# kmacrow/Shellac

Measured on AMD Instinct MI355X. Metric: cache_ops_per_s, higher is better.
Workload: dtype uint8

## Files before the change

shellac_amd/csrc/hbm_cache.h:

```cpp
#pragma once

#include <hip/hip_runtime_api.h>

#include <algorithm>
#include <mutex>
#include <string>
#include <vector>

#include "layout.h"

namespace shellac {

enum : int { kEvictFifo = 0, kEvictClock = 1 };

struct ShardConfig {
  uint64_t log_bytes = 1ull << 30;
  uint64_t nbuckets = 1ull << 20;
  uint32_t max_item = 1u << 20;
  int device = 0;
  int evict = kEvictClock;
  uint64_t reinsert_max = 0;
  int serve_blocks = 8;
};

// ... 117 lines not shown
  void ensure_set_ws(int64_t n, hipStream_t s);
  void ensure_rc_ws(int64_t w, hipStream_t s);
  void ensure_cb(int b, int64_t rows, hipStream_t s);
  bool should_reclaim(uint64_t bytes_bound) const;
  uint64_t* cur_ring_tail() const { return head_ + 2 + hsel_; }
  uint64_t* next_ring_tail() const { return head_ + 2 + (hsel_ ^ 1); }
  struct RetiredGroup {
    std::vector<void*> ptrs;
    std::vector<hipEvent_t> ev;
    uint64_t bytes = 0;
  };
  struct Buf {
    void** p;
    uint64_t (*bytes)(uint64_t cap);
  };
  using BufSet = std::vector<Buf>;
  void grow_bufs(const BufSet& set, int64_t old_cap, int64_t cap, hipStream_t s);
  void retire_group(const BufSet& set, int64_t cap, hipStream_t s);
  void reap_retired(bool all);
  void note_stream(hipStream_t s);
  void note_store_end(hipStream_t s);
  std::vector<RetiredGroup> retired_;
  uint64_t retired_ever_ = 0;
  struct SetStream {
    hipStream_t s = nullptr;
    hipEvent_t last = nullptr;
  };
  std::vector<SetStream> set_streams_;
  hipEvent_t ws_ready_ = nullptr;
  hipStream_t ws_grow_stream_ = nullptr;
  std::vector<hipStream_t> ws_ordered_;
  void ws_order(hipStream_t s);
  uint64_t* ring_ = nullptr;
  uint64_t ring_cap_ = 0;
  unsigned long long* rc_ctl_ = nullptr;
  bool lead_ = false;
  bool catch_up_ = true;
  uint64_t rmax_ = 0;
  int64_t rc_cap_ = 0;
  uint64_t *rc_loc_ = nullptr, *rc_h_ = nullptr, *rc_part_ = nullptr, *rc_hx_ = nullptr;
  BufSet rc_bufs();
  struct Pending {
    const Digest* keys = nullptr;
    const uint8_t* values = nullptr;
    const uint64_t* voff = nullptr;
    const uint32_t *vlen = nullptr, *flags = nullptr, *expire = nullptr;
    int64_t n = 0, rows = 0;
    const uint64_t* from = nullptr;
    int64_t nmove = 0;
    int ws = 0;
    int hand = -1;
    bool active = false;
  };
  Pending pend_;
  struct HandBuf {
    Digest* keys = nullptr;
    uint64_t* voff = nullptr;
    uint64_t* from = nullptr;
    uint32_t *vlen = nullptr, *flags = nullptr, *expire = nullptr;
    int64_t cap = 0;
    uint8_t* scratch = nullptr;
  };
  HandBuf hb_[2];
  static BufSet hand_bufs(HandBuf& h);
  struct SetWs {
    uint32_t* dd_tab = nullptr;
    uint32_t* dd_slot = nullptr;
    uint64_t *set_size = nullptr, *set_off = nullptr;
    uint32_t* set_claim = nullptr;
    uint64_t* set_cnt = nullptr;
  };
  SetWs ws_[2];
  int ws_next_ = 0;
  static BufSet set_bufs(SetWs& w);

  ShardConfig cfg_;
  uint8_t* log_ = nullptr;
  Entry* index_ = nullptr;
  uint64_t* head_ = nullptr;
  int hsel_ = 0;
  uint64_t* cur_head() const { return head_ + hsel_; }
  uint64_t* claim_ptr() const { return head_ + 4; }
  uint64_t* next_head() const { return head_ + (hsel_ ^ 1); }
  CacheCounters* ctr_ = nullptr;
  unsigned long long* scratch_ = nullptr;
  uint64_t* part_ = nullptr;
  uint64_t* host_buf_ = nullptr;
  uint64_t* host_slots_ = nullptr;
  void* srv_ring_ = nullptr;
  uint64_t* srv_ctl_ = nullptr;
  uint64_t* srv_sync_ = nullptr;
// ... 74 lines not shown
```

shellac_amd/csrc/hbm_cache.hip:

```cpp
#include <hip/hip_runtime.h>
#include <hip/hip_ext.h>
#include <hipcub/hipcub.hpp>

#include <algorithm>
#include <chrono>
#include <cstdlib>
#include <cstring>
#include <type_traits>
#include <vector>

#include "hbm_cache.h"
#include "keyed.h"
#include "trace.h"

namespace shellac {

#define HIP_OK(expr)                                                                   \
  do {                                                                                 \
    hipError_t _e = (expr);                                                            \
    if (_e != hipSuccess)                                                              \
      throw Error(std::string("HIP error ") + hipGetErrorString(_e) + " at " + #expr + \
                  " [" + __FILE__ + ":" + std::to_string(__LINE__) + "]");             \
  } while (0)

// ... 1647 lines not shown
    const uint64_t e2 = __shfl(w2[2], gbase + (target & 3));
    const uint64_t expected = target < 4 ? e1 : e2;
    Entry* const slot = index + (target < 4 ? b1 : b2) * kEntriesPerBucket + (target & 3);
    int ok = 0;
    if (l4 == 0) {
      const unsigned long long prev = atomicCAS(
          reinterpret_cast<unsigned long long*>(&slot->loc), (unsigned long long)expected,
          (unsigned long long)myloc);
      if (prev == expected) {
        slot->d0 = d.lo;
        slot->d1 = d.hi;
        *reinterpret_cast<uint64_t*>(&slot->vlen) = pack2(myvlen, myexp);
        *claim_out = (uint32_t)(slot - index);
        ok = 1;
        evicted += evict ? 1 : 0;
        bytes += myvlen;
      } else if (alt != ~0ull) {
        undo_relocation(index, alt, expected);
      }
    }
    ok = __shfl(ok, gbase);
    if (ok) break;
    if (attempt == 15 && l4 == 0) ++lost;
  }
}

__global__ __launch_bounds__(kBlock) __attribute__((amdgpu_waves_per_eu(8))) void k_set_index(
    const Digest* __restrict__ keys, int64_t n, const uint64_t* __restrict__ size,
    const uint64_t* __restrict__ off, const uint32_t* __restrict__ vlen,
    const uint32_t* __restrict__ expire, Entry* __restrict__ index, uint64_t mask,
    const uint64_t* __restrict__ head_ptr, uint64_t* __restrict__ head_next, uint64_t cap,
    uint32_t now, const uint32_t* __restrict__ slot_of, uint32_t* __restrict__ dd_tab,
    CacheCounters* __restrict__ ctr, uint32_t* __restrict__ claim,
    const uint64_t* __restrict__ from, int64_t r0, int64_t r1,
    const unsigned long long* __restrict__ r1_dev) {
  if (r1_dev && (int64_t)*r1_dev < r1) r1 = (int64_t)*r1_dev;
  const int l4 = threadIdx.x & 3;
  const int gbase = threadIdx.x & 60;
  const uint64_t base = *head_ptr;
  const uint64_t head_new = base + off[n];
  const int64_t ngroups = ((int64_t)gridDim.x * kBlock) >> 2;
  unsigned long long evicted = 0, bytes = 0, lost = 0, moved_away = 0;
  if (blockIdx.x == 0 && threadIdx.x == 0) *head_next = head_new;
  for (int64_t i = r0 + (((int64_t)blockIdx.x * kBlock + threadIdx.x) >> 2); i < r1; i += ngroups) {
    if (l4 == 0 && vlen[i] != kSkipVlen) dd_tab[slot_of[i]] = 0u;
    if (l4 == 0) claim[i] = ~0u;
    if (size[i] == 0) continue;
    const Digest d = keys[i];
    const uint64_t myloc = base + off[i] + 1;
    const uint32_t myvlen = vlen[i];
    const uint32_t myexp = expire ? expire[i] : 0u;
    const uint64_t fr = from ? from[i] : 0ull;
    const uint64_t b1 = bucket1(d, mask), b2 = bucket2(d, mask);
    const uint64_t* q1 = reinterpret_cast<const uint64_t*>(index + b1 * kEntriesPerBucket + l4);
    const uint64_t* q2 = reinterpret_cast<const uint64_t*>(index + b2 * kEntriesPerBucket + l4);
    for (int attempt = 0; attempt < 16; ++attempt) {
      uint64_t w1[4], w2[4];
#pragma unroll
      for (int k = 0; k < 4; ++k) {
        w1[k] = __hip_atomic_load(q1 + k, __ATOMIC_RELAXED, __HIP_MEMORY_SCOPE_AGENT);
        w2[k] = __hip_atomic_load(q2 + k, __ATOMIC_RELAXED, __HIP_MEMORY_SCOPE_AGENT);
      }
      const uint64_t span = head_new - base;
      const bool in1 = w1[2] - base - 1 < span || w1[2] == kLockedLoc;
      const bool in2 = w2[2] - base - 1 < span || w2[2] == kLockedLoc;
      const bool m1 = w1[0] == d.lo && w1[1] == d.hi && !in1;
      const bool m2 = w2[0] == d.lo && w2[1] == d.hi && !in2;
      const bool v1 = !entry_free(w1[2], (uint32_t)(w1[3] >> 32), head_new, cap, now);
      const bool v2 = !entry_free(w2[2], (uint32_t)(w2[3] >> 32), head_new, cap, now);
      const uint32_t mmask = (uint32_t)((__ballot(m1) >> gbase) & 0xfull) |
                             ((uint32_t)((__ballot(m2) >> gbase) & 0xfull) << 4);
      const uint32_t lmask = (uint32_t)((__ballot(v1) >> gbase) & 0xfull) |
                             ((uint32_t)((__ballot(v2) >> gbase) & 0xfull) << 4);
      int target;
      if (fr) {
        const uint32_t fmask = (uint32_t)((__ballot(w1[2] == fr) >> gbase) & 0xfull) |
                               ((uint32_t)((__ballot(w2[2] == fr) >> gbase) & 0xfull) << 4);
        if (!fmask) {
          if (l4 == 0) ++moved_away;
          break;
        }
        target = __ffs(fmask) - 1;
      } else if (mmask) {
        target = __ffs(mmask) - 1;
      } else {
        const uint32_t dead = ~lmask & 0xffu;
        if (dead) {
          const int live1 = __popc(lmask & 0xfu), live2 = __popc(lmask & 0xf0u);
          const uint32_t pref = __popc(dead & 0x0fu) >= 2
                                    ? (dead & 0x0fu)
                                    : (live2 < live1 ? (dead & 0xf0u) : (dead & 0x0fu));
          target = __ffs(pref ? pref : dead) - 1;
        } else {
          if (l4 == 0) claim[i] = kClaimDeferred;
          break;
        }
      }
      const uint64_t e1 = __shfl(w1[2], gbase + (target & 3));
      const uint64_t e2 = __shfl(w2[2], gbase + (target & 3));
      const uint64_t expected = target < 4 ? e1 : e2;
      Entry* const slot = index + (target < 4 ? b1 : b2) * kEntriesPerBucket + (target & 3);
      int ok = 0;
// ... 68 lines not shown
          const uint64_t aw = agent_load(reinterpret_cast<const uint64_t*>(&a->vlen));
          if (!entry_free(al, (uint32_t)(aw >> 32), head_new, cap, now)) continue;
          if (copy_entry(a, al, de.lo, de.hi, l, w)) {
            target = x;
            expected = l;
            copy = a;
          }
          break;
        }
      }
      if (!target && victim) {
        target = victim;
        expected = oldest;
        evict = true;
      }
    }
    if (!target) continue;
    if (copy_entry(target, expected, d.lo, d.hi, myloc, myword)) {
      *claim_out = (uint32_t)(target - index);
      evicted += evict ? 1 : 0;
      bytes += (uint32_t)myword;
      return;
    }
    if (copy) drop_entry(copy, expected);
  }
  ++lost;
}

__global__ __launch_bounds__(kBlock) void k_set_fixup(
    const Digest* __restrict__ keys, int64_t n, const uint64_t* __restrict__ off,
    const uint32_t* __restrict__ vlen, const uint32_t* __restrict__ expire,
    const uint64_t* __restrict__ head_ptr, uint32_t* __restrict__ claim,
    Entry* __restrict__ index, const uint64_t* __restrict__ size, uint64_t* __restrict__ ring,
    uint64_t rmask, const uint64_t* __restrict__ ring_tail, uint64_t* __restrict__ ring_tail_next,
    const uint64_t* __restrict__ cnt_off, uint64_t* __restrict__ head_host, uint64_t mask,
    uint64_t cap, uint32_t now, CacheCounters* __restrict__ ctr) {
  const uint64_t base = *head_ptr;
  const uint64_t rtail = ring ? *ring_tail : 0;
  if (blockIdx.x == 0 && threadIdx.x == 0) {
    if (ring) *ring_tail_next = rtail + cnt_off[n];
    if (head_host)
      __hip_atomic_store(head_host, base + off[n], __ATOMIC_RELAXED, __HIP_MEMORY_SCOPE_SYSTEM);
  }
  if (ring)
    for (int64_t i = (int64_t)blockIdx.x * kBlock + threadIdx.x; i < n;
         i += (int64_t)gridDim.x * kBlock)
      if (size[i]) ring[(rtail + cnt_off[i]) & rmask] = base + off[i] + 0;
  unsigned long long evicted = 0, lost = 0, bytes = 0;
  for (int64_t i = (int64_t)blockIdx.x * kBlock + threadIdx.x; i < n;
       i += (int64_t)gridDim.x * kBlock) {
    if (!size[i]) continue;
    uint32_t c = claim[i];
    if (c == kClaimDeferred) {
      claim[i] = ~0u;
      deferred_insert(keys[i], base + off[i] + 1, pack2(vlen[i], expire ? expire[i] : 0u), index,
                      mask, base, off[n], base + off[n], cap, now, claim + i, evicted, bytes,
                      lost);
      continue;
    }
    if (c == ~0u) continue;
    Entry* const e = index + c;
    if (e->loc != base + off[i] + 1) continue;
    const Digest d = keys[i];
    uint64_t* const ew = reinterpret_cast<uint64_t*>(&e->vlen);
    const uint64_t w = pack2(vlen[i], expire ? expire[i] : 0u);
    const uint64_t e0 = e->d0, e1 = e->d1, e3 = *ew;
    if (e0 != d.lo) e->d0 = d.lo;
    if (e1 != d.hi) e->d1 = d.hi;
    if ((e3 & ~(uint64_t)kRefBit) != w) *ew = w;
  }
  block_count(ctr, evicted, &CacheCounters::set_evicted, lost, &CacheCounters::set_dropped, bytes,
              &CacheCounters::set_bytes);
}

constexpr int kSmallSetRows = kBlock;
constexpr int kSetSmallU = 16;

__global__ __launch_bounds__(kBlock) void k_set_small(
    const Digest* __restrict__ keys, const uint8_t* __restrict__ values,
    const uint64_t* __restrict__ val_off, const uint32_t* __restrict__ vlen,
    const uint32_t* __restrict__ flags, const uint32_t* __restrict__ expire, int n,
    uint32_t max_item, Entry* __restrict__ index, uint64_t mask,
    const uint64_t* __restrict__ head_ptr, uint64_t* __restrict__ head_next,
    unsigned long long* __restrict__ claim_word, uint64_t cap, uint32_t now,
    uint8_t* __restrict__ log, uint64_t* __restrict__ ring, uint64_t rmask,
    const uint64_t* __restrict__ ring_tail, uint64_t* __restrict__ ring_tail_next,
    uint64_t* __restrict__ head_host, CacheCounters* __restrict__ ctr) {
  constexpr int kT = 2 * kSmallSetRows;
  __shared__ unsigned long long s_tk[kT];
  __shared__ int s_tw[kT];
  __shared__ uint64_t s_off[kSmallSetRows + 1];
  __shared__ uint64_t s_src[kSmallSetRows];
  __shared__ uint32_t s_cnt[kSmallSetRows + 1];
  __shared__ uint32_t s_claim[kSmallSetRows];
  __shared__ Digest s_key[kSmallSetRows];
  __shared__ uint32_t s_vl[kSmallSetRows];
  __shared__ uint32_t s_ex[kSmallSetRows];
  __shared__ unsigned long long s_w[2][kBlock / 64];
  const int tid = threadIdx.x, lane = tid & 63, w = tid >> 6;
  for (int k = tid; k < kT; k += kBlock) {
    s_tk[k] = 0ull;
    s_tw[k] = -1;
  }
  __syncthreads();
  const bool row = tid < n;
  const uint32_t vl = row ? vlen[tid] : kSkipVlen;
  const bool skip = vl == kSkipVlen;
  Digest d{0, 0};
  int slot = -1;
  s_vl[tid] = vl;
  s_ex[tid] = row && expire ? expire[tid] : 0u;
  if (row && !skip) {
    d = keys[tid];
    s_key[tid] = d;
    const unsigned long long key = d.lo ? d.lo : 1ull;
    uint32_t t = (uint32_t)fmix64(key) & (kT - 1);
    for (int probe = 0; probe < kT; ++probe) {
      const unsigned long long prev = atomicCAS(&s_tk[t], 0ull, key);
      if (prev == 0ull || prev == key) {
        atomicMax(&s_tw[t], tid);
// ... 82 lines not shown
      if (dst[u]) *reinterpret_cast<u32x4*>(dst[u]) = v[u];
  }
  asm volatile("s_waitcnt vmcnt(0)" ::: "memory");
  __syncthreads();
  if (tid == 0) {
    __builtin_amdgcn_fence(__ATOMIC_RELEASE, "agent");
    asm volatile("s_waitcnt vmcnt(0)" ::: "memory");
  }
  __syncthreads();
  unsigned long long evicted = 0, bytes = 0, lost = 0;
  for (int i0 = 0; i0 < n; i0 += kBlock / 4) {
    const int i = i0 + (tid >> 2);
    const bool act = i < n && s_off[i + 1] != s_off[i];
    if ((tid & 3) == 0 && i < n) s_claim[i] = ~0u;
    index_insert(act, act ? s_key[i] : Digest{0, 0}, base + s_off[i] + 1, act ? s_vl[i] : 0u,
                 act ? s_ex[i] : 0u, s_claim + (i < n ? i : 0), index, mask, base, head_new,
                 cap, now, evicted, bytes, lost);
  }
  asm volatile("s_waitcnt vmcnt(0)" ::: "memory");
  __syncthreads();
  if (row && win) {
    const uint32_t c = s_claim[tid];
    const uint64_t myloc = base + my_off + 1;
    if (c != ~0u) {
      Entry* const e = index + c;
      if (__hip_atomic_load(&e->loc, __ATOMIC_RELAXED, __HIP_MEMORY_SCOPE_AGENT) == myloc) {
        e->d0 = d.lo;
        e->d1 = d.hi;
        *reinterpret_cast<uint64_t*>(&e->vlen) = pack2(vl, s_ex[tid]);
      }
    }
  }
  const uint64_t rtail = ring ? *ring_tail : 0;
  if (ring && row && win) ring[(rtail + s_cnt[tid]) & rmask] = base + my_off;
  if (tid == 0) {
    *head_next = head_new;
    if (ring) *ring_tail_next = rtail + s_cnt[kSmallSetRows];
    __hip_atomic_store(head_host, head_new, __ATOMIC_RELAXED, __HIP_MEMORY_SCOPE_SYSTEM);
  }
  block_count(ctr, (unsigned long long)(row && !skip ? 1 : 0), &CacheCounters::set_ops,
              (unsigned long long)(row && !skip && !win ? 1 : 0), &CacheCounters::set_dropped);
  block_count(ctr, evicted, &CacheCounters::set_evicted, bytes, &CacheCounters::set_bytes, lost,
              &CacheCounters::set_dropped);
}

constexpr unsigned long long kRcCount = 1ull << 43;
constexpr int kRcScanK = 1;

struct RcArgs {
  const uint64_t* ring;
  uint64_t rmask;
  const uint64_t* ring_tail;
  unsigned long long* ctl;
  int64_t W;
  int64_t n_new;
  int parity;
  const uint64_t* head_ptr;
  uint64_t cap;
  uint32_t now;
  uint64_t rmax;
  uint64_t lead_mode;
};

struct RcBatch {
  Digest* keys;
  uint64_t* voff;
  uint32_t* vlen;
  uint32_t* flags;
  uint32_t* expire;
  uint64_t* from;
};

__device__ __forceinline__ void block_partial_at(unsigned long long v, uint64_t* __restrict__ part,
                                                 int64_t at) {
  __shared__ unsigned long long s_p[kBlock / 64];
  v = wave_sum(v);
  if ((threadIdx.x & 63) == 0) s_p[threadIdx.x >> 6] = v;
  __syncthreads();
  if (threadIdx.x == 0) {
    unsigned long long t = 0;
#pragma unroll
    for (int k = 0; k < kBlock / 64; ++k) t += s_p[k];
    part[at] = t;
  }
  __syncthreads();
}

template <int K>
__global__ __launch_bounds__(kBlock) void k_rc_scan(RcArgs a, RcBatch cb, const uint8_t* __restrict__ log,
                                                    const Entry* __restrict__ index, uint64_t mask,
                                                    const Digest* __restrict__ keys,
                                                    const uint8_t* __restrict__ values,
                                                    const uint64_t* __restrict__ val_off,
                                                    const uint32_t* __restrict__ vlen_new,
                                                    const uint32_t* __restrict__ flags,
                                                    const uint32_t* __restrict__ expire,
                                                    int64_t n_new, uint32_t max_item,
                                                    uint64_t* __restrict__ rc_loc,
                                                    uint64_t* __restrict__ rc_h,
                                                    uint64_t* __restrict__ part_h) {
  const uint64_t hand = a.ctl[0], rtail = *a.ring_tail, head = *a.head_ptr;
  unsigned long long best = 0;
  for (int64_t i = (int64_t)blockIdx.x * kBlock + threadIdx.x; i < n_new;
       i += (int64_t)gridDim.x * kBlock) {
    const uint32_t v = vlen_new[i];
    if (v != kSkipVlen && v <= max_item) best += item_bytes(v);
    const int64_t r = a.W + i;
    cb.keys[r] = keys[i];
    cb.voff[r] = (uint64_t)(uintptr_t)values + val_off[i];
    cb.vlen[r] = v;
    cb.flags[r] = flags ? flags[i] : 0u;
    cb.expire[r] = expire ? expire[i] : 0u;
    cb.from[r] = 0;
  }
  const uint64_t avail = rtail - hand;
  const int64_t weff = hand_window_eff(a.n_new, a.ctl[4]);
  if (blockIdx.x == 0 && threadIdx.x == 0) {
    a.ctl[3] = (uint64_t)weff < avail ? (uint64_t)weff : avail;
    a.ctl[5 + a.parity] = (unsigned long long)weff;
  }
  int64_t j[K];
  uint64_t l[K], loc[K], h[K];
  uint4 w0[K], w1[K];
#pragma unroll
  for (int k = 0; k < K; ++k) {
    j[k] = ((int64_t)blockIdx.x * K + k) * kBlock + threadIdx.x;
    l[k] = kRingSkip;
    loc[k] = kRingSkip;
    h[k] = 0;
    w0[k] = w1[k] = make_uint4(0, 0, 0, 0);
    if (j[k] < weff && (uint64_t)j[k] < avail) {
      const uint64_t idx = hand + (uint64_t)j[k];
      l[k] = rtail - idx <= a.rmask + 1 ? a.ring[idx & a.rmask] : kRingSkip;
    }
  }
#pragma unroll
  for (int k = 0; k < K; ++k)
    if (l[k] != kRingSkip && head <= l[k] + a.cap) {
      const uint4* hp = reinterpret_cast<const uint4*>(log + l[k] % a.cap);
      w0[k] = hp[0];
      w1[k] = hp[1];
    }
  uint4 hv[K][kEntriesPerBucket];
  bool found[K];
#pragma unroll
  for (int k = 0; k < K; ++k) {
    found[k] = false;
    if (l[k] != kRingSkip && w1[k].w == kItemMagic) {
      loc[k] = l[k];
      const Digest d{pack2(w0[k].x, w0[k].y), pack2(w0[k].z, w0[k].w)};
      const uint64_t b = bucket1(d, mask);
#pragma unroll
      for (int e = 0; e < (int)kEntriesPerBucket; ++e)
        hv[k][e] = reinterpret_cast<const uint4*>(index + b * kEntriesPerBucket + e)[1];
    }
  }
#pragma unroll
  for (int k = 0; k < K; ++k) {
    if (loc[k] == kRingSkip) continue;
#pragma unroll
    for (int e = 0; e < (int)kEntriesPerBucket; ++e)
      if (pack2(hv[k][e].x, hv[k][e].y) == loc[k] + 1) {
        found[k] = true;
        if ((hv[k][e].z & kRefBit) && (hv[k][e].w == 0 || hv[k][e].w > a.now))
          h[k] = item_bytes(w1[k].x);
      }
    if (!found[k]) {
      const Digest d{pack2(w0[k].x, w0[k].y), pack2(w0[k].z, w0[k].w)};
      const uint64_t b = bucket2(d, mask);
      uint4 h2[kEntriesPerBucket];
#pragma unroll
      for (int e = 0; e < (int)kEntriesPerBucket; ++e)
        h2[e] = reinterpret_cast<const uint4*>(index + b * kEntriesPerBucket + e)[1];
#pragma unroll
      for (int e = 0; e < (int)kEntriesPerBucket; ++e)
        if (pack2(h2[e].x, h2[e].y) == loc[k] + 1) {
          if ((h2[e].z & kRefBit) && (h2[e].w == 0 || h2[e].w > a.now)) h[k] = item_bytes(w1[k].x);
        }
    }
  }
#pragma unroll
  for (int k = 0; k < K; ++k) {
    if (j[k] >= weff && j[k] < a.W) {
      cb.vlen[j[k]] = kSkipVlen;
    } else if (j[k] < a.W) {
      rc_loc[j[k]] = loc[k];
      rc_h[j[k]] = h[k];
      cb.keys[j[k]] = h[k] ? Digest{pack2(w0[k].x, w0[k].y), pack2(w0[k].z, w0[k].w)} : Digest{0, 0};
      cb.voff[j[k]] = 0;
      cb.vlen[j[k]] = h[k] ? w1[k].x : kSkipVlen;
      cb.flags[j[k]] = h[k] ? w1[k].y : 0u;
      cb.expire[j[k]] = h[k] ? w1[k].z : 0u;
      cb.from[j[k]] = 0;
    }
    block_partial_at(h[k] ? h[k] + kRcCount : 0ull, part_h, (int64_t)blockIdx.x * K + k);
  }
  __shared__ unsigned long long s_b[kBlock / 64];
  best = wave_sum(best);
  if ((threadIdx.x & 63) == 0) s_b[threadIdx.x >> 6] = best;
  __syncthreads();
  if (threadIdx.x == 0) {
    unsigned long long t = 0;
#pragma unroll
    for (int k = 0; k < kBlock / 64; ++k) t += s_b[k];
    if (t) atomicAdd(&a.ctl[1], t);
  }
}

__global__ __launch_bounds__(kBlock) void k_rc_emit(RcArgs a, RcBatch cb,
                                                    const uint8_t* __restrict__ log,
                                                    uint64_t* __restrict__ rc_loc,
                                                    uint64_t* __restrict__ rc_h,
                                                    const uint64_t* __restrict__ part_h,
                                                    uint64_t* __restrict__ rc_hx,
                                                    const uint8_t* __restrict__ scratch,
                                                    CacheCounters* __restrict__ ctr) {
  __shared__ unsigned long long s_w[kBlock / 64];
  __shared__ unsigned long long s_pre;
  if (a.lead_mode && (uint64_t)blockIdx.x * kBlock >= a.ctl[3]) return;
  const int lane = threadIdx.x & 63, w = threadIdx.x >> 6;
  unsigned long long pre = 0;
  for (unsigned b = threadIdx.x; b < blockIdx.x; b += kBlock) pre += part_h[b];
  pre = wave_sum(pre);
  if (lane == 0) s_w[w] = pre;
  __syncthreads();
  if (threadIdx.x == 0) s_pre = s_w[0] + s_w[1] + s_w[2] + s_w[3];
// ... 743 lines not shown
  HIP_OK(hipHostMalloc(&host_slots_, kHostSlots * sizeof(uint64_t),
                       hipHostMallocMapped | hipHostMallocCoherent));
  memset(host_slots_, 0, kHostSlots * sizeof(uint64_t));
  SH_CHECK(cfg_.serve_blocks >= 1 && cfg_.serve_blocks <= kServeBlocksMax,
           "serve_blocks out of range");
  srv_blocks_ = cfg_.serve_blocks;
  HIP_OK(hipHostMalloc(&srv_ring_, (size_t)kServeRing * srv_blocks_ * sizeof(SrvJob),
                       hipHostMallocMapped | hipHostMallocCoherent));
  memset(srv_ring_, 0, (size_t)kServeRing * srv_blocks_ * sizeof(SrvJob));
  HIP_OK(hipHostMalloc(&srv_ctl_, kCtlWords * sizeof(uint64_t),
                       hipHostMallocMapped | hipHostMallocCoherent));
  memset(srv_ctl_, 0, kCtlWords * sizeof(uint64_t));
  HIP_OK(hipMalloc(&srv_sync_, 64));
  HIP_OK(hipHostMalloc(&srv_trace_, kSrvTrace * 8 * sizeof(uint64_t),
                       hipHostMallocMapped | hipHostMallocCoherent));
  memset(srv_trace_, 0, kSrvTrace * 8 * sizeof(uint64_t));
  {
    int khz = 0;
    HIP_OK(hipDeviceGetAttribute(&khz, hipDeviceAttributeWallClockRate, cfg_.device));
    if (khz <= 0) khz = 100000;
    srv_khz_ = (uint64_t)khz;
    srv_idle_ticks_ = (uint64_t)khz * kSrvIdleUs / 1000;
    srv_life_ticks_ = (uint64_t)khz * kSrvLifeUs / 1000;
  }
  HIP_OK(hipMemset(index_, 0, cfg_.nbuckets * kBucketBytes));
  HIP_OK(hipMemset(head_, 0, 64));
  HIP_OK(hipMemset(ctr_, 0, kCtrShards * sizeof(CacheCounters)));
  SH_CHECK(cfg_.evict == kEvictFifo || cfg_.evict == kEvictClock, "unknown eviction policy");
  SH_CHECK(cfg_.max_item <= kVlenMask, "max_item must be < 2 GiB (CLOCK bit in vlen)");
  if (cfg_.evict == kEvictClock) {
    rmax_ = reinsert_budget(cfg_.log_bytes, cfg_.reinsert_max);
    ring_cap_ = ring_entries(cfg_.nbuckets);
    HIP_OK(hipMalloc(&ring_, ring_cap_ * sizeof(uint64_t)));
    HIP_OK(hipMalloc(&rc_ctl_, 8 * sizeof(unsigned long long)));
    HIP_OK(hipMemset(rc_ctl_, 0, 8 * sizeof(unsigned long long)));
    HIP_OK(hipMemset(rc_ctl_ + 2, 0xff, sizeof(unsigned long long)));
    for (HandBuf& b : hb_) HIP_OK(hipMalloc(&b.scratch, rmax_ + 64));
  }
  HIP_OK(hipDeviceSynchronize());
}

HbmCache::~HbmCache() {
  DeviceGuard g(cfg_.device);
  try {
    serve_stop();
  } catch (...) {
  }
  (void)hipDeviceSynchronize();
  if (srv_stream_) (void)hipStreamDestroy(srv_stream_);
  (void)hipHostFree(srv_ring_);
  (void)hipHostFree(srv_ctl_);
  (void)hipHostFree(srv_trace_);
  (void)hipFree(srv_sync_);
  (void)hipFree(log_);
  (void)hipFree(index_);
  (void)hipFree(head_);
  (void)hipFree(ctr_);
  (void)hipFree(scratch_);
  (void)hipFree(done_ctr_);
  (void)hipFree(lb_state_);
  (void)hipFree(part_);
  (void)hipHostFree(host_buf_);
  (void)hipHostFree(host_slots_);
  (void)hipFree(ring_); (void)hipFree(rc_ctl_);
  const auto free_bufs = [](const BufSet& set) {
    for (const Buf& b : set) (void)hipFree(*b.p);
  };
  free_bufs(rc_bufs());
  for (SetWs& w : ws_) free_bufs(set_bufs(w));
  for (HandBuf& h : hb_) {
    free_bufs(hand_bufs(h));
    (void)hipFree(h.scratch);
  }
  reap_retired(true);
  if (ws_ready_) (void)hipEventDestroy(ws_ready_);
  for (const SetStream& x : set_streams_)
    if (x.last) (void)hipEventDestroy(x.last);
}

#define SH_BUF(ptr, expr) \
  Buf { reinterpret_cast<void**>(&(ptr)), [](uint64_t cap) -> uint64_t { return expr; } }
HbmCache::BufSet HbmCache::set_bufs(SetWs& w) {
  return {SH_BUF(w.dd_tab, 2 * cap * sizeof(uint32_t)),
          SH_BUF(w.dd_slot, cap * sizeof(uint32_t)),
          SH_BUF(w.set_size, (cap + 1) * sizeof(uint64_t)),
          SH_BUF(w.set_off, (cap + 1) * sizeof(uint64_t)),
          SH_BUF(w.set_claim, cap * sizeof(uint32_t)),
          SH_BUF(w.set_cnt, (cap + 1) * sizeof(uint64_t))};
}
HbmCache::BufSet HbmCache::hand_bufs(HandBuf& h) {
  return {SH_BUF(h.keys, cap * sizeof(Digest)), SH_BUF(h.voff, cap * 8),
          SH_BUF(h.from, cap * 8),              SH_BUF(h.vlen, cap * 4),
          SH_BUF(h.flags, cap * 4),             SH_BUF(h.expire, cap * 4)};
}
HbmCache::BufSet HbmCache::rc_bufs() {
  return {SH_BUF(rc_loc_, cap * 8), SH_BUF(rc_h_, cap * 8),
          SH_BUF(rc_part_, (cap / kBlock + 5) * 8),
          SH_BUF(rc_hx_, (cap + 1) * 8)};
}
#undef SH_BUF

void HbmCache::grow_bufs(const BufSet& set, int64_t old_cap, int64_t cap, hipStream_t s) {
  retire_group(set, old_cap, s);
  for (const Buf& b : set) HIP_OK(hipMalloc(b.p, b.bytes((uint64_t)cap)));
}

namespace {
int64_t grown_cap(int64_t cap, int64_t want, int64_t first) {
  int64_t c = cap ? cap : first;
  while (c < want) c *= 2;
  return c;
}
}

void HbmCache::retire_group(const BufSet& set, int64_t cap, hipStream_t s) {
  RetiredGroup g;
  for (const Buf& b : set)
    if (*b.p) {
      g.ptrs.push_back(*b.p);
      g.bytes += b.bytes((uint64_t)cap);
    }
  if (g.ptrs.empty()) return;
  retired_ever_ += g.bytes;
  for (const SetStream& x : set_streams_)
    if (x.s != s && x.last) HIP_OK(hipStreamWaitEvent(s, x.last, 0));
  hipEvent_t e;
// ... 24 lines not shown
  DeviceGuard g(cfg_.device);
  reap_retired(false);
  uint64_t b = 0;
  for (const RetiredGroup& r : retired_) b += r.bytes;
  return b;
}

void HbmCache::ws_order(hipStream_t s) {
  if (!ws_ready_ || s == ws_grow_stream_) return;
  if (std::find(ws_ordered_.begin(), ws_ordered_.end(), s) != ws_ordered_.end()) return;
  HIP_OK(hipStreamWaitEvent(s, ws_ready_, 0));
  ws_ordered_.push_back(s);
}

void HbmCache::note_stream(hipStream_t s) {
  for (const SetStream& x : set_streams_)
    if (x.s == s) return;
  SetStream x;
  x.s = s;
  HIP_OK(hipEventCreateWithFlags(&x.last, hipEventDisableTiming | hipEventDisableSystemFence));
  set_streams_.push_back(x);
}

void HbmCache::note_store_end(hipStream_t s) {
  for (const SetStream& x : set_streams_)
    if (x.s == s) {
      (void)hipEventRecord(x.last, s);
      return;
    }
}

uint64_t HbmCache::hbm_bytes() const {
  return cfg_.log_bytes + item_bytes(cfg_.max_item) + 64 + cfg_.nbuckets * kBucketBytes +
         ring_cap_ * sizeof(uint64_t) + (hb_[0].scratch ? 2 * (rmax_ + 64) : 0);
}

void HbmCache::ensure_rc_ws(int64_t w, hipStream_t s) {
  if (w <= rc_cap_) return;
  const int64_t cap = grown_cap(rc_cap_, w, 4096);
  grow_bufs(rc_bufs(), rc_cap_, cap, s);
  rc_cap_ = cap;
}

void HbmCache::ensure_cb(int b, int64_t rows, hipStream_t s) {
  HandBuf& h = hb_[b];
  if (rows <= h.cap) return;
  const int64_t cap = grown_cap(h.cap, rows, 4096);
  grow_bufs(hand_bufs(h), h.cap, cap, s);
  h.cap = cap;
}

bool HbmCache::should_reclaim(uint64_t bytes_bound) const {
  if (cfg_.evict != kEvictClock) return false;
  const uint64_t h = __atomic_load_n(host_slots_ + kHeadSlot, __ATOMIC_ACQUIRE);
  return h + 4 * (bytes_bound + rmax_) > cfg_.log_bytes;
}

HbmCache::Pending HbmCache::reclaim_locked(const Pending& own, int64_t w, uint64_t rmax,
                                           uint32_t now, hipStream_t s, bool detached) {
  RcArgs a{ring_, ring_cap_ - 1, detached ? next_ring_tail() : cur_ring_tail(), rc_ctl_, w,
           own.n, own.hand, claim_ptr(), cfg_.log_bytes, now, rmax, lead_ ? 1ull : 0ull};
  const int g = (int)((w + kBlock - 1) / kBlock);
  const HandBuf& hb = hb_[own.hand];
  const RcBatch cb{hb.keys, hb.voff, hb.vlen, hb.flags, hb.expire, hb.from};
  static const int rk = [] {
    const char* e = getenv("SHELLAC_RCSCAN_K");
    const int v = e ? atoi(e) : kRcScanK;
    return v == 1 || v == 2 || v == 4 ? v : kRcScanK;
  }();
  auto scan = k_rc_scan<4>;
  if (rk == 2) scan = k_rc_scan<2>;
  if (rk == 1) scan = k_rc_scan<1>;
  hipLaunchKernelGGL(scan, dim3((g + rk - 1) / rk), dim3(kBlock), 0, s, a, cb, log_, index_,
                     cfg_.nbuckets - 1, own.keys, own.values, own.voff, own.vlen, own.flags,
                     own.expire, own.n, cfg_.max_item, rc_loc_, rc_h_, rc_part_);
  hipLaunchKernelGGL(k_rc_emit, dim3(g), dim3(kBlock), 0, s, a, cb, log_, rc_loc_, rc_h_,
                     rc_part_, rc_hx_, hb.scratch, ctr_);
  if (!lead_)
    launch_segcopy<2>(s, log_, rc_loc_, rc_hx_, w, hb.scratch, nullptr, nullptr, nullptr,
                      nullptr, rc_h_, rmax);
  HIP_OK(hipGetLastError());
  return Pending{hb.keys, nullptr, hb.voff,  hb.vlen, hb.flags, hb.expire,
                 own.n,   w + own.n, hb.from, w,      own.ws,   own.hand};
}

void HbmCache::ensure_set_ws(int64_t n, hipStream_t s) {
  if (n <= set_cap_) return;
  const int64_t cap = grown_cap(set_cap_, n, 1024);
  for (SetWs& w : ws_) {
    grow_bufs(set_bufs(w), set_cap_, cap, s);
    HIP_OK(hipMemsetAsync(w.dd_tab, 0, (size_t)cap * 2 * sizeof(uint32_t), s));
  }
  dd_mask_ = (uint32_t)(cap * 2 - 1);
  set_cap_ = cap;
  ++ws_gen_;
  if (!ws_ready_) HIP_OK(hipEventCreateWithFlags(&ws_ready_, hipEventDisableTiming));
  HIP_OK(hipEventRecord(ws_ready_, s));
  ws_grow_stream_ = s;
  ws_ordered_.clear();
}

void HbmCache::reserve(int64_t n) {
  std::lock_guard<std::mutex> lk(mu_);
  DeviceGuard g(cfg_.device);
  if (cfg_.evict == kEvictClock && rmax_ && n > 0) {
    const int64_t w = hand_window(n);
    ensure_rc_ws(w, nullptr);
    ensure_cb(0, w + n, nullptr);
    ensure_cb(1, w + n, nullptr);
    n = w + n;
  }
  ensure_set_ws(n, nullptr);
  HIP_OK(hipDeviceSynchronize());
  reap_retired(true);
}

// ... 283 lines not shown
  }
  SH_CHECK(bytes_bound <= cfg_.log_bytes / 2,
           "SET batch larger than half the log; split the batch");
  std::lock_guard<std::mutex> lk(mu_);
  DeviceGuard g(cfg_.device);
  note_stream(s);
  struct EndMark {
    HbmCache* c;
    hipStream_t s;
    hipEvent_t done;
    ~EndMark() {
      if (done) (void)hipEventRecord(done, s);
      c->note_store_end(s);
    }
  } end_mark{this, s, o.done};
  if (!retired_.empty()) reap_retired(false);
  Pending p{keys, values, val_off, vlen, flags, expire, n, n};
  if (o.phase == 2) {
    SH_CHECK(pend_.active && pend_.n == n, "store phase 2 without the same batch's phase 1");
    p = pend_;
    pend_.active = false;
  } else {
    SH_CHECK(!pend_.active, "store: a phase-1 batch is still waiting for its phase 2");
    const uint64_t rmax =
        std::min<uint64_t>(rmax_, cfg_.log_bytes / 2 - bytes_bound) / 16 * 16;
    const bool hand = o.allow_reclaim && rmax && should_reclaim(bytes_bound);
    lead_ = hand_lead(cfg_.log_bytes, bytes_bound, rmax, lead_);
    if (!hand && o.phase == 0 && n <= kSmallSetRows && !o.index_after && !o.append_after &&
        !o.append_done && !o.plan_done) {
      hipLaunchKernelGGL(k_set_small, dim3(1), dim3(kBlock), 0, s, keys, values, val_off, vlen,
                         flags, expire, (int)n, cfg_.max_item, index_, cfg_.nbuckets - 1,
                         cur_head(), next_head(),
                         reinterpret_cast<unsigned long long*>(claim_ptr()), cfg_.log_bytes,
                         now, log_, ring_, ring_ ? ring_cap_ - 1 : 0ull, cur_ring_tail(),
                         next_ring_tail(), host_slots_ + kHeadSlot, ctr_);
      HIP_OK(hipGetLastError());
      hsel_ ^= 1;
      return;
    }
    p.ws = ws_next_;
    ws_next_ ^= 1;
    const bool detached = o.phase == 1;
    if (hand) {
      const int64_t w = hand_window(n);
      p.hand = p.ws;
      ensure_rc_ws(w, s);
      ensure_cb(p.hand, w + n, s);
      ensure_set_ws(w + n, s);
      p = reclaim_locked(p, w, rmax, now, s, detached);
    } else {
      ensure_set_ws(n, s);
    }
    ws_order(s);
    store_plan_locked(p, s, detached);
    if (o.plan_done) HIP_OK(hipEventRecord(o.plan_done, s));
    if (detached) {
      pend_ = p;
      pend_.active = true;
      return;
    }
  }
  store_tail_locked(p, now, s, o, &end_mark.done);
  hsel_ ^= 1;
}

void HbmCache::store_tail_locked(const Pending& p, uint32_t now, hipStream_t s,
                                 const StoreOpts& o, hipEvent_t* done) {
  if (o.append_after) HIP_OK(hipStreamWaitEvent(s, o.append_after, 0));
// ... 6 lines not shown

void HbmCache::store_plan_locked(const Pending& p, hipStream_t s, bool detached) {
  const SetWs& w = ws_[p.ws];
  const int64_t n = p.rows;
  const int grid = grid_for(n, kBlock, kMaxGrid);
  RcAdvance adv;
  if (p.nmove > 0)
    adv = RcAdvance{rc_ctl_, detached ? next_ring_tail() : cur_ring_tail(), ring_cap_ - 1,
                    p.nmove, ring_, claim_ptr(), cfg_.log_bytes, catch_up_ ? 1 : 0};
  hipLaunchKernelGGL(k_set_dedupe, dim3(grid), dim3(kBlock), 0, s, p.keys, p.vlen, n, w.dd_tab,
                     dd_mask_, w.dd_slot, adv);
  const int sgrid = grid_for(n, kBlock, kMaxGrid);
  uint64_t* part_cnt = ring_ ? part_ + 2 * kMaxGrid : nullptr;
  hipLaunchKernelGGL(k_set_size, dim3(sgrid), dim3(kBlock), 0, s, p.vlen, n, w.dd_tab,
                     w.dd_slot, cfg_.max_item, w.set_size, ctr_, part_ + kMaxGrid, part_cnt);
  HIP_OK(hipGetLastError());
  launch_offsets(w.set_size, n, part_ + kMaxGrid, sgrid, w.set_off, s, nullptr, 0, part_cnt,
                 ring_ ? w.set_cnt : nullptr, detached ? claim_ptr() : cur_head(),
                 claim_ptr());
}

void HbmCache::store_index_locked(const Pending& p, uint32_t now, hipStream_t s,
                                  hipEvent_t index_after, hipEvent_t* done) {
  const SetWs& w = ws_[p.ws];
  const int64_t n = p.rows;
  if (index_after) HIP_OK(hipStreamWaitEvent(s, index_after, 0));
  for (int pass = p.nmove > 0 ? 0 : 1; pass < 2; ++pass) {
    const int64_t r0 = pass ? p.nmove : 0, r1 = pass ? n : p.nmove;
    if (r1 <= r0) continue;
    const int igrid = grid_for((r1 - r0) * 4, kBlock, kMaxGrid);
    hipLaunchKernelGGL(k_set_index, dim3(igrid), dim3(kBlock), 0, s, p.keys, n, w.set_size,
                       w.set_off, p.vlen, p.expire, index_, cfg_.nbuckets - 1, cur_head(),
                       next_head(), cfg_.log_bytes, now, w.dd_slot, w.dd_tab, ctr_, w.set_claim,
                       pass ? (const uint64_t*)nullptr : p.from, r0, r1,
                       pass ? nullptr : rc_ctl_ + 5 + p.hand);
  }
  launch_stop(done, k_set_fixup, dim3(grid_for(n, kBlock, kMaxGrid)), dim3(kBlock), s, p.keys,
              n, w.set_off, p.vlen, p.expire, cur_head(), w.set_claim, index_, w.set_size,
              ring_, ring_ ? ring_cap_ - 1 : 0ull, cur_ring_tail(), next_ring_tail(), w.set_cnt,
              host_slots_ + kHeadSlot, cfg_.nbuckets - 1, cfg_.log_bytes, now, ctr_);
  HIP_OK(hipGetLastError());
}

void HbmCache::destroy_graph(StoreGraph* g) {
  for (auto& e : g->exec)
    if (e) {
      (void)hipGraphExecDestroy(e);
      e = nullptr;
    }
  g->n = -1;
}

void HbmCache::store_graph(StoreGraph* g, const Digest* keys, const uint8_t* values,
                           const uint64_t* val_off, const uint32_t* vlen, const uint32_t* flags,
                           const uint32_t* expire, int64_t n, uint64_t bytes_bound,
                           uint32_t now, hipStream_t s) {
  TraceRange tr("hbm.store_graph");
  if (n <= 0) return;
  SH_CHECK(s != nullptr, "store_graph needs a created stream (the legacy default stream "
                         "cannot be captured)");
  SH_CHECK(bytes_bound <= cfg_.log_bytes / 2,
           "SET batch larger than half the log; split the batch");
  std::lock_guard<std::mutex> lk(mu_);
  DeviceGuard dg(cfg_.device);
  ensure_set_ws(n, s);
  ws_order(s);
  const Pending b{keys, values, val_off, vlen, flags, expire, n, n};
  const void* ptrs[6] = {keys, values, val_off, vlen, flags, expire};
  bool same = g->n == n && g->bound == bytes_bound && g->now == now && g->ws_gen == ws_gen_ &&
              g->exec[0] && g->exec[1];
  for (int i = 0; same && i < 6; ++i) same = g->ptrs[i] == ptrs[i];
  if (!same) {
    destroy_graph(g);
// ... 287 lines not shown
```

Baseline: 3.668 billion.

## Store index slot hints in the ring to skip bucket probes during reclaim

Adds a per-ring-entry slot hint array recording where each item landed in the index. The reclaim scan first checks the hinted bucket and reads the log header only for hot or unlocated items. Moved items are reinserted by CAS directly at their known slot instead of re-probing both cuckoo buckets. The fixup kernel drops its entry-rewrite tail and writes ring and hint together. The cost is an extra 4 bytes of HBM per ring slot, and stale hints fall back to the full probe.

Result: no change. 3.640 billion (-0.8%).

```diff
diff --git a/shellac_amd/csrc/hbm_cache.h b/shellac_amd/csrc/hbm_cache.h
--- a/shellac_amd/csrc/hbm_cache.h
+++ b/shellac_amd/csrc/hbm_cache.h
@@ -173,6 +173,7 @@
   std::vector<hipStream_t> ws_ordered_;
   void ws_order(hipStream_t s);
   uint64_t* ring_ = nullptr;
+  uint32_t* ring_hint_ = nullptr;
   uint64_t ring_cap_ = 0;
   unsigned long long* rc_ctl_ = nullptr;
   bool lead_ = false;
@@ -188,6 +189,7 @@
     const uint32_t *vlen = nullptr, *flags = nullptr, *expire = nullptr;
     int64_t n = 0, rows = 0;
     const uint64_t* from = nullptr;
+    const uint32_t* slot = nullptr;
     int64_t nmove = 0;
     int ws = 0;
     int hand = -1;
@@ -198,6 +200,7 @@
     Digest* keys = nullptr;
     uint64_t* voff = nullptr;
     uint64_t* from = nullptr;
+    uint32_t* slot = nullptr;
     uint32_t *vlen = nullptr, *flags = nullptr, *expire = nullptr;
     int64_t cap = 0;
     uint8_t* scratch = nullptr;
diff --git a/shellac_amd/csrc/hbm_cache.hip b/shellac_amd/csrc/hbm_cache.hip
--- a/shellac_amd/csrc/hbm_cache.hip
+++ b/shellac_amd/csrc/hbm_cache.hip
@@ -1703,8 +1703,8 @@
     const uint64_t* __restrict__ head_ptr, uint64_t* __restrict__ head_next, uint64_t cap,
     uint32_t now, const uint32_t* __restrict__ slot_of, uint32_t* __restrict__ dd_tab,
     CacheCounters* __restrict__ ctr, uint32_t* __restrict__ claim,
-    const uint64_t* __restrict__ from, int64_t r0, int64_t r1,
-    const unsigned long long* __restrict__ r1_dev) {
+    const uint64_t* __restrict__ from, const uint32_t* __restrict__ from_slot, int64_t r0,
+    int64_t r1, const unsigned long long* __restrict__ r1_dev) {
   if (r1_dev && (int64_t)*r1_dev < r1) r1 = (int64_t)*r1_dev;
   const int l4 = threadIdx.x & 3;
   const int gbase = threadIdx.x & 60;
@@ -1722,6 +1722,21 @@
     const uint32_t myvlen = vlen[i];
     const uint32_t myexp = expire ? expire[i] : 0u;
     const uint64_t fr = from ? from[i] : 0ull;
+    if (fr) {
+      int ok = 0;
+      const uint32_t fs = from_slot[i];
+      if (l4 == 0 && fs < (uint32_t)((mask + 1) * kEntriesPerBucket)) {
+        Entry* const slot = index + fs;
+        if (atomicCAS(reinterpret_cast<unsigned long long*>(&slot->loc), (unsigned long long)fr,
+                      (unsigned long long)myloc) == fr) {
+          *reinterpret_cast<uint64_t*>(&slot->vlen) = pack2(myvlen, myexp);
+          claim[i] = fs;
+          bytes += myvlen;
+          ok = 1;
+        }
+      }
+      if (__shfl(ok, gbase)) continue;
+    }
     const uint64_t b1 = bucket1(d, mask), b2 = bucket2(d, mask);
     const uint64_t* q1 = reinterpret_cast<const uint64_t*>(index + b1 * kEntriesPerBucket + l4);
     const uint64_t* q2 = reinterpret_cast<const uint64_t*>(index + b2 * kEntriesPerBucket + l4);
@@ -1737,8 +1752,8 @@
       const bool in2 = w2[2] - base - 1 < span || w2[2] == kLockedLoc;
       const bool m1 = w1[0] == d.lo && w1[1] == d.hi && !in1;
       const bool m2 = w2[0] == d.lo && w2[1] == d.hi && !in2;
-      const bool v1 = !entry_free(w1[2], (uint32_t)(w1[3] >> 32), head_new, cap, now);
-      const bool v2 = !entry_free(w2[2], (uint32_t)(w2[3] >> 32), head_new, cap, now);
+      const bool v1 = in1 || !entry_free(w1[2], (uint32_t)(w1[3] >> 32), head_new, cap, now);
+      const bool v2 = in2 || !entry_free(w2[2], (uint32_t)(w2[3] >> 32), head_new, cap, now);
       const uint32_t mmask = (uint32_t)((__ballot(m1) >> gbase) & 0xfull) |
                              ((uint32_t)((__ballot(m2) >> gbase) & 0xfull) << 4);
       const uint32_t lmask = (uint32_t)((__ballot(v1) >> gbase) & 0xfull) |
@@ -1873,9 +1888,10 @@
     const uint32_t* __restrict__ vlen, const uint32_t* __restrict__ expire,
     const uint64_t* __restrict__ head_ptr, uint32_t* __restrict__ claim,
     Entry* __restrict__ index, const uint64_t* __restrict__ size, uint64_t* __restrict__ ring,
-    uint64_t rmask, const uint64_t* __restrict__ ring_tail, uint64_t* __restrict__ ring_tail_next,
-    const uint64_t* __restrict__ cnt_off, uint64_t* __restrict__ head_host, uint64_t mask,
-    uint64_t cap, uint32_t now, CacheCounters* __restrict__ ctr) {
+    uint32_t* __restrict__ ring_hint, uint64_t rmask, const uint64_t* __restrict__ ring_tail,
+    uint64_t* __restrict__ ring_tail_next, const uint64_t* __restrict__ cnt_off,
+    uint64_t* __restrict__ head_host, uint64_t mask, uint64_t cap, uint32_t now,
+    CacheCounters* __restrict__ ctr) {
   const uint64_t base = *head_ptr;
   const uint64_t rtail = ring ? *ring_tail : 0;
   if (blockIdx.x == 0 && threadIdx.x == 0) {
@@ -1883,10 +1899,6 @@
     if (head_host)
       __hip_atomic_store(head_host, base + off[n], __ATOMIC_RELAXED, __HIP_MEMORY_SCOPE_SYSTEM);
   }
-  if (ring)
-    for (int64_t i = (int64_t)blockIdx.x * kBlock + threadIdx.x; i < n;
-         i += (int64_t)gridDim.x * kBlock)
-      if (size[i]) ring[(rtail + cnt_off[i]) & rmask] = base + off[i] + 0;
   unsigned long long evicted = 0, lost = 0, bytes = 0;
   for (int64_t i = (int64_t)blockIdx.x * kBlock + threadIdx.x; i < n;
        i += (int64_t)gridDim.x * kBlock) {
@@ -1897,18 +1909,13 @@
       deferred_insert(keys[i], base + off[i] + 1, pack2(vlen[i], expire ? expire[i] : 0u), index,
                       mask, base, off[n], base + off[n], cap, now, claim + i, evicted, bytes,
                       lost);
-      continue;
-    }
-    if (c == ~0u) continue;
-    Entry* const e = index + c;
-    if (e->loc != base + off[i] + 1) continue;
-    const Digest d = keys[i];
-    uint64_t* const ew = reinterpret_cast<uint64_t*>(&e->vlen);
-    const uint64_t w = pack2(vlen[i], expire ? expire[i] : 0u);
-    const uint64_t e0 = e->d0, e1 = e->d1, e3 = *ew;
-    if (e0 != d.lo) e->d0 = d.lo;
-    if (e1 != d.hi) e->d1 = d.hi;
-    if ((e3 & ~(uint64_t)kRefBit) != w) *ew = w;
+      c = claim[i];
+    }
+    if (ring) {
+      const uint64_t r = (rtail + cnt_off[i]) & rmask;
+      ring[r] = base + off[i];
+      ring_hint[r] = c;
+    }
   }
   block_count(ctr, evicted, &CacheCounters::set_evicted, lost, &CacheCounters::set_dropped, bytes,
               &CacheCounters::set_bytes);
@@ -1924,9 +1931,10 @@
     uint32_t max_item, Entry* __restrict__ index, uint64_t mask,
     const uint64_t* __restrict__ head_ptr, uint64_t* __restrict__ head_next,
     unsigned long long* __restrict__ claim_word, uint64_t cap, uint32_t now,
-    uint8_t* __restrict__ log, uint64_t* __restrict__ ring, uint64_t rmask,
-    const uint64_t* __restrict__ ring_tail, uint64_t* __restrict__ ring_tail_next,
-    uint64_t* __restrict__ head_host, CacheCounters* __restrict__ ctr) {
+    uint8_t* __restrict__ log, uint64_t* __restrict__ ring, uint32_t* __restrict__ ring_hint,
+    uint64_t rmask, const uint64_t* __restrict__ ring_tail,
+    uint64_t* __restrict__ ring_tail_next, uint64_t* __restrict__ head_host,
+    CacheCounters* __restrict__ ctr) {
   constexpr int kT = 2 * kSmallSetRows;
   __shared__ unsigned long long s_tk[kT];
   __shared__ int s_tw[kT];
@@ -2075,7 +2083,10 @@
     }
   }
   const uint64_t rtail = ring ? *ring_tail : 0;
-  if (ring && row && win) ring[(rtail + s_cnt[tid]) & rmask] = base + my_off;
+  if (ring && row && win) {
+    ring[(rtail + s_cnt[tid]) & rmask] = base + my_off;
+    ring_hint[(rtail + s_cnt[tid]) & rmask] = s_claim[tid];
+  }
   if (tid == 0) {
     *head_next = head_new;
     if (ring) *ring_tail_next = rtail + s_cnt[kSmallSetRows];
@@ -2092,6 +2103,7 @@
 
 struct RcArgs {
   const uint64_t* ring;
+  const uint32_t* ring_hint;
   uint64_t rmask;
   const uint64_t* ring_tail;
   unsigned long long* ctl;
@@ -2112,6 +2124,7 @@
   uint32_t* flags;
   uint32_t* expire;
   uint64_t* from;
+  uint32_t* slot;
 };
 
 __device__ __forceinline__ void block_partial_at(unsigned long long v, uint64_t* __restrict__ part,
@@ -2164,53 +2177,76 @@
   }
   int64_t j[K];
   uint64_t l[K], loc[K], h[K];
+  uint32_t hint[K], slot[K];
   uint4 w0[K], w1[K];
+  const uint32_t nslots = (uint32_t)((mask + 1) * kEntriesPerBucket);
 #pragma unroll
   for (int k = 0; k < K; ++k) {
     j[k] = ((int64_t)blockIdx.x * K + k) * kBlock + threadIdx.x;
     l[k] = kRingSkip;
     loc[k] = kRingSkip;
     h[k] = 0;
+    hint[k] = slot[k] = ~0u;
     w0[k] = w1[k] = make_uint4(0, 0, 0, 0);
     if (j[k] < weff && (uint64_t)j[k] < avail) {
       const uint64_t idx = hand + (uint64_t)j[k];
-      l[k] = rtail - idx <= a.rmask + 1 ? a.ring[idx & a.rmask] : kRingSkip;
-    }
+      if (rtail - idx <= a.rmask + 1) {
+        l[k] = a.ring[idx & a.rmask];
+        hint[k] = a.ring_hint[idx & a.rmask];
+      }
+    }
+    if (l[k] != kRingSkip && head > l[k] + a.cap) l[k] = kRingSkip;
+  }
+  uint4 hv[K][kEntriesPerBucket];
+  bool found[K], hot[K];
+#pragma unroll
+  for (int k = 0; k < K; ++k) {
+    found[k] = hot[k] = false;
+    if (l[k] != kRingSkip && hint[k] < nslots) {
+      const Entry* const b = index + (hint[k] & ~(uint32_t)(kEntriesPerBucket - 1));
+#pragma unroll
+      for (int e = 0; e < (int)kEntriesPerBucket; ++e)
+        hv[k][e] = reinterpret_cast<const uint4*>(b + e)[1];
+    } else {
+#pragma unroll
+      for (int e = 0; e < (int)kEntriesPerBucket; ++e) hv[k][e] = make_uint4(0, 0, 0, 0);
+    }
+  }
+#pragma unroll
+  for (int k = 0; k < K; ++k) {
+    if (l[k] == kRingSkip || hint[k] >= nslots) continue;
+#pragma unroll
+    for (int e = 0; e < (int)kEntriesPerBucket; ++e)
+      if (pack2(hv[k][e].x, hv[k][e].y) == l[k] + 1) {
+        found[k] = true;
+        slot[k] = (hint[k] & ~(uint32_t)(kEntriesPerBucket - 1)) + e;
+        if ((hv[k][e].z & kRefBit) && (hv[k][e].w == 0 || hv[k][e].w > a.now)) hot[k] = true;
+      }
   }
 #pragma unroll
   for (int k = 0; k < K; ++k)
-    if (l[k] != kRingSkip && head <= l[k] + a.cap) {
+    if (l[k] != kRingSkip && (hot[k] || !found[k])) {
       const uint4* hp = reinterpret_cast<const uint4*>(log + l[k] % a.cap);
       w0[k] = hp[0];
       w1[k] = hp[1];
     }
-  uint4 hv[K][kEntriesPerBucket];
-  bool found[K];
 #pragma unroll
   for (int k = 0; k < K; ++k) {
-    found[k] = false;
-    if (l[k] != kRingSkip && w1[k].w == kItemMagic) {
-      loc[k] = l[k];
-      const Digest d{pack2(w0[k].x, w0[k].y), pack2(w0[k].z, w0[k].w)};
-      const uint64_t b = bucket1(d, mask);
-#pragma unroll
-      for (int e = 0; e < (int)kEntriesPerBucket; ++e)
-        hv[k][e] = reinterpret_cast<const uint4*>(index + b * kEntriesPerBucket + e)[1];
-    }
-  }
-#pragma unroll
-  for (int k = 0; k < K; ++k) {
-    if (loc[k] == kRingSkip) continue;
-#pragma unroll
-    for (int e = 0; e < (int)kEntriesPerBucket; ++e)
-      if (pack2(hv[k][e].x, hv[k][e].y) == loc[k] + 1) {
-        found[k] = true;
-        if ((hv[k][e].z & kRefBit) && (hv[k][e].w == 0 || hv[k][e].w > a.now))
-          h[k] = item_bytes(w1[k].x);
-      }
-    if (!found[k]) {
-      const Digest d{pack2(w0[k].x, w0[k].y), pack2(w0[k].z, w0[k].w)};
-      const uint64_t b = bucket2(d, mask);
+    if (l[k] == kRingSkip) continue;
+    if (found[k]) {
+      if (!hot[k]) loc[k] = l[k];
+      else if (w1[k].w == kItemMagic) {
+        loc[k] = l[k];
+        h[k] = item_bytes(w1[k].x);
+      }
+      continue;
+    }
+    if (w1[k].w != kItemMagic) continue;
+    loc[k] = l[k];
+    const Digest d{pack2(w0[k].x, w0[k].y), pack2(w0[k].z, w0[k].w)};
+#pragma unroll 1
+    for (int side = 0; side < 2 && !found[k]; ++side) {
+      const uint64_t b = side ? bucket2(d, mask) : bucket1(d, mask);
       uint4 h2[kEntriesPerBucket];
 #pragma unroll
       for (int e = 0; e < (int)kEntriesPerBucket; ++e)
@@ -2218,6 +2254,8 @@
 #pragma unroll
       for (int e = 0; e < (int)kEntriesPerBucket; ++e)
         if (pack2(h2[e].x, h2[e].y) == loc[k] + 1) {
+          found[k] = true;
+          slot[k] = (uint32_t)(b * kEntriesPerBucket + e);
           if ((h2[e].z & kRefBit) && (h2[e].w == 0 || h2[e].w > a.now)) h[k] = item_bytes(w1[k].x);
         }
     }
@@ -2235,6 +2273,7 @@
       cb.flags[j[k]] = h[k] ? w1[k].y : 0u;
       cb.expire[j[k]] = h[k] ? w1[k].z : 0u;
       cb.from[j[k]] = 0;
+      cb.slot[j[k]] = slot[k];
     }
     block_partial_at(h[k] ? h[k] + kRcCount : 0ull, part_h, (int64_t)blockIdx.x * K + k);
   }
@@ -3044,6 +3083,8 @@
     rmax_ = reinsert_budget(cfg_.log_bytes, cfg_.reinsert_max);
     ring_cap_ = ring_entries(cfg_.nbuckets);
     HIP_OK(hipMalloc(&ring_, ring_cap_ * sizeof(uint64_t)));
+    HIP_OK(hipMalloc(&ring_hint_, ring_cap_ * sizeof(uint32_t)));
+    HIP_OK(hipMemset(ring_hint_, 0xff, ring_cap_ * sizeof(uint32_t)));
     HIP_OK(hipMalloc(&rc_ctl_, 8 * sizeof(unsigned long long)));
     HIP_OK(hipMemset(rc_ctl_, 0, 8 * sizeof(unsigned long long)));
     HIP_OK(hipMemset(rc_ctl_ + 2, 0xff, sizeof(unsigned long long)));
@@ -3074,7 +3115,7 @@
   (void)hipFree(part_);
   (void)hipHostFree(host_buf_);
   (void)hipHostFree(host_slots_);
-  (void)hipFree(ring_); (void)hipFree(rc_ctl_);
+  (void)hipFree(ring_); (void)hipFree(ring_hint_); (void)hipFree(rc_ctl_);
   const auto free_bufs = [](const BufSet& set) {
     for (const Buf& b : set) (void)hipFree(*b.p);
   };
@@ -3103,7 +3144,8 @@
 HbmCache::BufSet HbmCache::hand_bufs(HandBuf& h) {
   return {SH_BUF(h.keys, cap * sizeof(Digest)), SH_BUF(h.voff, cap * 8),
           SH_BUF(h.from, cap * 8),              SH_BUF(h.vlen, cap * 4),
-          SH_BUF(h.flags, cap * 4),             SH_BUF(h.expire, cap * 4)};
+          SH_BUF(h.flags, cap * 4),             SH_BUF(h.expire, cap * 4),
+          SH_BUF(h.slot, cap * 4)};
 }
 HbmCache::BufSet HbmCache::rc_bufs() {
   return {SH_BUF(rc_loc_, cap * 8), SH_BUF(rc_h_, cap * 8),
@@ -3194,7 +3236,7 @@
 
 uint64_t HbmCache::hbm_bytes() const {
   return cfg_.log_bytes + item_bytes(cfg_.max_item) + 64 + cfg_.nbuckets * kBucketBytes +
-         ring_cap_ * sizeof(uint64_t) + (hb_[0].scratch ? 2 * (rmax_ + 64) : 0);
+         ring_cap_ * (sizeof(uint64_t) + sizeof(uint32_t)) + (hb_[0].scratch ? 2 * (rmax_ + 64) : 0);
 }
 
 void HbmCache::ensure_rc_ws(int64_t w, hipStream_t s) {
@@ -3220,11 +3262,11 @@
 
 HbmCache::Pending HbmCache::reclaim_locked(const Pending& own, int64_t w, uint64_t rmax,
                                            uint32_t now, hipStream_t s, bool detached) {
-  RcArgs a{ring_, ring_cap_ - 1, detached ? next_ring_tail() : cur_ring_tail(), rc_ctl_, w,
+  RcArgs a{ring_, ring_hint_, ring_cap_ - 1, detached ? next_ring_tail() : cur_ring_tail(), rc_ctl_, w,
            own.n, own.hand, claim_ptr(), cfg_.log_bytes, now, rmax, lead_ ? 1ull : 0ull};
   const int g = (int)((w + kBlock - 1) / kBlock);
   const HandBuf& hb = hb_[own.hand];
-  const RcBatch cb{hb.keys, hb.voff, hb.vlen, hb.flags, hb.expire, hb.from};
+  const RcBatch cb{hb.keys, hb.voff, hb.vlen, hb.flags, hb.expire, hb.from, hb.slot};
   static const int rk = [] {
     const char* e = getenv("SHELLAC_RCSCAN_K");
     const int v = e ? atoi(e) : kRcScanK;
@@ -3242,8 +3284,8 @@
     launch_segcopy<2>(s, log_, rc_loc_, rc_hx_, w, hb.scratch, nullptr, nullptr, nullptr,
                       nullptr, rc_h_, rmax);
   HIP_OK(hipGetLastError());
-  return Pending{hb.keys, nullptr, hb.voff,  hb.vlen, hb.flags, hb.expire,
-                 own.n,   w + own.n, hb.from, w,      own.ws,   own.hand};
+  return Pending{hb.keys, nullptr,   hb.voff, hb.vlen, hb.flags, hb.expire, own.n,
+                 w + own.n, hb.from, hb.slot, w,      own.ws,   own.hand};
 }
 
 void HbmCache::ensure_set_ws(int64_t n, hipStream_t s) {
@@ -3593,8 +3635,8 @@
                          flags, expire, (int)n, cfg_.max_item, index_, cfg_.nbuckets - 1,
                          cur_head(), next_head(),
                          reinterpret_cast<unsigned long long*>(claim_ptr()), cfg_.log_bytes,
-                         now, log_, ring_, ring_ ? ring_cap_ - 1 : 0ull, cur_ring_tail(),
-                         next_ring_tail(), host_slots_ + kHeadSlot, ctr_);
+                         now, log_, ring_, ring_hint_, ring_ ? ring_cap_ - 1 : 0ull,
+                         cur_ring_tail(), next_ring_tail(), host_slots_ + kHeadSlot, ctr_);
       HIP_OK(hipGetLastError());
       hsel_ ^= 1;
       return;
@@ -3667,13 +3709,13 @@
     hipLaunchKernelGGL(k_set_index, dim3(igrid), dim3(kBlock), 0, s, p.keys, n, w.set_size,
                        w.set_off, p.vlen, p.expire, index_, cfg_.nbuckets - 1, cur_head(),
                        next_head(), cfg_.log_bytes, now, w.dd_slot, w.dd_tab, ctr_, w.set_claim,
-                       pass ? (const uint64_t*)nullptr : p.from, r0, r1,
+                       pass ? (const uint64_t*)nullptr : p.from, p.slot, r0, r1,
                        pass ? nullptr : rc_ctl_ + 5 + p.hand);
   }
   launch_stop(done, k_set_fixup, dim3(grid_for(n, kBlock, kMaxGrid)), dim3(kBlock), s, p.keys,
               n, w.set_off, p.vlen, p.expire, cur_head(), w.set_claim, index_, w.set_size,
-              ring_, ring_ ? ring_cap_ - 1 : 0ull, cur_ring_tail(), next_ring_tail(), w.set_cnt,
-              host_slots_ + kHeadSlot, cfg_.nbuckets - 1, cfg_.log_bytes, now, ctr_);
+              ring_, ring_hint_, ring_ ? ring_cap_ - 1 : 0ull, cur_ring_tail(), next_ring_tail(),
+              w.set_cnt, host_slots_ + kHeadSlot, cfg_.nbuckets - 1, cfg_.log_bytes, now, ctr_);
   HIP_OK(hipGetLastError());
 }
 
```
